# mayataka/robotoc

Measured on NVIDIA H100. Metric: SQP-iterations/s (ANYmal N=40, batch=1024) at 1/2/4/8 H100 vs CPU ref, higher is better.
Workload: dtype f64

## Files before the change

robotoc_b200/csrc/riccati_forward.cuh:

```cuda
#pragma once
#include "rbt_device.cuh"
#include "../../include/rbt_layout.h"

namespace rbt {

struct FwdParams {
  rbt_layout L;
  const rbt_stage_ctrl* ctrl;
  int n_grid;
  int batch;
  const double* kkt;
  const double* ric;
  const double* dx0;
  double* dir;
  int segs;
  const double* dxseed;
  const int* tp_fail;
};

template <int NV, int NU, int NS>
struct FwdCfg {
  static constexpr int NX = 2 * NV;
  static constexpr int NTHREADS = 96;
  static constexpr int KPART = NX * NX + ((NV * NU + 1) & ~1) + ((NX + 1) & ~1);
  static constexpr int RPART = NX * NX + ((NX + 1) & ~1) + ((NU * NX + 1) & ~1) + ((NU + 1) & ~1);
  static constexpr int e_M = 0;
  static constexpr int e_m = e_M + ((NS * NX + 1) & ~1);
  static constexpr int e_Psi = e_m + ((NS + 1) & ~1);
  static constexpr int e_Phi = e_Psi + ((NX + 1) & ~1);
  static constexpr int e_T = e_Phi + ((NX + 1) & ~1);
  static constexpr int e_W = e_T + ((NU + 1) & ~1);
  static constexpr int e_mt = e_W + ((NU + 1) & ~1);
  static constexpr int e_mtn = e_mt + ((NS + 1) & ~1);
  static constexpr int e_pol = e_mtn + ((NS + 1) & ~1);
  static constexpr int e_fx = e_pol + ((NX + 1) & ~1) + 2;
  static constexpr int ESZ = e_fx + ((NX + 1) & ~1);
  static constexpr int SLOT = KPART + RPART + ESZ;
  static constexpr int o_dx = 2 * SLOT;
  static constexpr int o_du = o_dx + 2 * NX;
  static constexpr int o_sc = o_du + ((NU + 1) & ~1);
  static constexpr int o_bar = o_sc + 4;
  static constexpr int SMEM_DOUBLES = o_bar + 4;
  static constexpr size_t SMEM_BYTES = size_t(SMEM_DOUBLES) * 8;
};

template <int NV, int NU, int NS, bool SEG = false>
__global__ void __launch_bounds__(FwdCfg<NV, NU, NS>::NTHREADS, 3) riccati_forward_kernel(const FwdParams p) {
  using C = FwdCfg<NV, NU, NS>;
  constexpr int NX = C::NX, NTHR = C::NTHREADS;
  constexpr int CO = ((NX + 15) / 16) * 16;
  static_assert(CO + NX <= NTHR, "costate thread group must fit");
  extern __shared__ __align__(16) double smem[];
  const rbt_layout& L = p.L;
  const int tid = threadIdx.x;
  const int b = SEG ? int(blockIdx.x) / p.segs : int(blockIdx.x);
  if (b >= p.batch) return;
  const int N = p.n_grid - 1;
  int lo = 0, last = N, seg = 0;
  if constexpr (SEG) {
    seg = int(blockIdx.x) % p.segs;
    if (p.tp_fail[b] != 0) {
      if (seg != 0) return;
    } else {
      lo = tp_seg_lo(seg, N, p.segs);
      last = (seg == p.segs - 1) ? N : tp_seg_lo(seg + 1, N, p.segs) - 1;
    }
  }
  const double* kkt_b = p.kkt + size_t(b) * p.n_grid * L.k_stride;
  const double* ric_b = p.ric + size_t(b) * p.n_grid * L.r_stride;
  double* dir_b = p.dir + size_t(b) * p.n_grid * L.d_stride;
  double* sdx = smem + C::o_dx;
  double* sdu = smem + C::o_du;
  double* ssc = smem + C::o_sc;
  uint64_t* bars = reinterpret_cast<uint64_t*>(smem + C::o_bar);

  auto needs_pol = [&](int st) {
    const rbt_stage_ctrl c = p.ctrl[st];
    return (st == 0 && c.sto) || ((c.type == RBT_IMPACT || c.type == RBT_LIFT) && c.sto_next);
  };
  auto has_extras = [&](int st) {
    const rbt_stage_ctrl c = p.ctrl[st];
    return c.ns > 0 || c.sto || needs_pol(st);
  };
  auto issue = [&](int st) {
    const int slot = (st - lo) & 1;
    double* base = smem + slot * C::SLOT;
    const rbt_stage_ctrl c = p.ctrl[st];
    const double* krec = kkt_b + size_t(st) * L.k_stride;
    const double* rrec = ric_b + size_t(st) * L.r_stride;
    fence_proxy_async();
    if (st < N) {
      mbar_expect_tx(&bars[slot], uint32_t(C::KPART + C::RPART) * 8u);
      tma_load_1d(base, krec + L.k_Fxx, uint32_t(C::KPART) * 8u, &bars[slot]);
      tma_load_1d(base + C::KPART, rrec + L.r_P, uint32_t(C::RPART) * 8u, &bars[slot]);
    } else {
      const uint32_t by = uint32_t(NX * NX + ((NX + 1) & ~1)) * 8u;
      mbar_expect_tx(&bars[slot], by);
      tma_load_1d(base + C::KPART, rrec + L.r_P, by, &bars[slot]);
    }
    if (st < N && has_extras(st)) {
      double* ex = base + C::KPART + C::RPART;
      uint32_t bytes = 0;
      if (c.ns > 0) bytes += uint32_t(C::e_Psi - C::e_M) * 8u;
      if (c.sto) bytes += uint32_t(C::e_mt - C::e_Psi) * 8u + uint32_t(C::ESZ - C::e_fx) * 8u;
      if (c.sto && c.ns > 0) bytes += uint32_t(C::e_pol - C::e_mt) * 8u;
      if (needs_pol(st)) bytes += uint32_t(C::e_fx - C::e_pol) * 8u;
      mbar_expect_tx(&bars[2 + slot], bytes);
      if (c.ns > 0) tma_load_1d(ex + C::e_M, rrec + L.r_M, uint32_t(C::e_Psi - C::e_M) * 8u, &bars[2 + slot]);
      if (c.sto) {
        tma_load_1d(ex + C::e_Psi, rrec + L.r_Psi, uint32_t(C::e_mt - C::e_Psi) * 8u, &bars[2 + slot]);
        tma_load_1d(ex + C::e_fx, krec + L.k_fx, uint32_t(C::ESZ - C::e_fx) * 8u, &bars[2 + slot]);
      }
      if (c.sto && c.ns > 0) tma_load_1d(ex + C::e_mt, rrec + L.r_mt, uint32_t(C::e_pol - C::e_mt) * 8u, &bars[2 + slot]);
      if (needs_pol(st)) tma_load_1d(ex + C::e_pol, rrec + L.r_dtsdx, uint32_t(C::e_fx - C::e_pol) * 8u, &bars[2 + slot]);
    }
  };

  if (tid == 0) {
    for (int q = 0; q < 4; ++q) mbar_init(&bars[q], 1);
    fence_mbar_init();
  }
  if (tid < NX) sdx[tid] = (SEG && lo > 0) ? p.dxseed[(size_t(b) * p.segs + seg) * NX + tid] : p.dx0[size_t(b) * NX + tid];
  if (tid == 0) {
    ssc[0] = 0.0;
    ssc[1] = 0.0;
  }
  __syncthreads();
  if (tid == 0) {
    issue(lo);
    if (last >= lo + 1) issue(lo + 1);
  }
  uint32_t pe0 = 0, pe1 = 0;

  for (int i = lo; i <= last; ++i) {
    const int slot = (i - lo) & 1;
    const rbt_stage_ctrl c = p.ctrl[i];
    const double* base = smem + slot * C::SLOT;
    const double* sA = base;
    const double* sB = base + NX * NX;
    const double* sFx = sB + ((NV * NU + 1) & ~1);
    const double* sPm = base + C::KPART;
    const double* ss = sPm + NX * NX;
    const double* sKt = ss + ((NX + 1) & ~1);
    const double* sk = sKt + ((NU * NX + 1) & ~1);
    const double* ex = base + C::KPART + C::RPART;
    double* dx = sdx + ((i - lo) & 1) * NX;
    double* dxn = sdx + ((i - lo + 1) & 1) * NX;
    double* drec = dir_b + size_t(i) * L.d_stride;
    const bool terminal = (i == N);
    const bool impact = (!terminal && c.type == RBT_IMPACT);
    const bool lift = (!terminal && c.type == RBT_LIFT);
    const bool sto = !terminal && c.sto, sto_next = !terminal && c.sto_next;
    const bool extras = !terminal && has_extras(i);

    mbar_wait(&bars[slot], uint32_t((i - lo) >> 1) & 1u);
    if (extras) {
      if (slot) {
        mbar_wait(&bars[3], pe1);
        pe1 ^= 1;
      } else {
        mbar_wait(&bars[2], pe0);
        pe0 ^= 1;
      }
    }

    double dts = ssc[0], dtsn = ssc[1];
    if (i == 0 && sto) {
      dtsn = dot_serial(ex + C::e_pol, dx, NX) + ex[C::e_pol + ((NX + 1) & ~1) + 1];
    }
    if (lift) {
      dts = dtsn;
      dtsn = 0.0;
      if (sto_next) {
        dtsn = dot_serial(ex + C::e_pol, dx, NX) + ex[C::e_pol + ((NX + 1) & ~1) + 1];
        if (sto) dtsn += ex[C::e_pol + ((NX + 1) & ~1)] * dts;
      }
    }
    if (impact) {
      dts = dtsn;
      dtsn = 0.0;
    }
    const double delta = dtsn - dts;

    if (!terminal && !impact) {
      matvec_T(sKt, NX, NX, NU, dx, tid, NTHR, [&](int u, double a) {
        double v = a + sk[u];
        if (sto) {
          v += ex[C::e_T + u] * delta;
          if (sto_next) v -= ex[C::e_W + u] * dtsn;
        }
        sdu[u] = v;
        drec[L.d_du + u] = v;
      });
      __syncthreads();
    }
    if (tid < NX) {
      const int r = tid;
      drec[L.d_dx + r] = dx[r];
      if (!terminal) {
        double a = sFx[r];
        for (int k = 0; k < NX; ++k) a = fma(sA[r + k * NX], dx[k], a);
        if (!impact) {
          if (r >= NV)
            for (int u = 0; u < NU; ++u) a = fma(sB[(r - NV) + u * NV], sdu[u], a);
          if (sto) a = fma(ex[C::e_fx + r], delta, a);
        }
        dxn[r] = a;
      }
    } else if (tid >= CO && tid < CO + NX && !(impact && sto_next)) {
      const int r = tid - CO;
      double a = -ss[r];
      for (int k = 0; k < NX; ++k) a = fma(sPm[r + k * NX], dx[k], a);
      if (sto) {
        if (impact) {
          a -= ex[C::e_Phi + r] * dtsn;
        } else {
          a += ex[C::e_Psi + r] * delta;
          if (sto_next) a -= ex[C::e_Phi + r] * dtsn;
        }
      }
      drec[L.d_dlmdgmm + r] = a;
    }
    __syncthreads();

    if (impact && sto_next) {
      const double e_dts = dts;
      double e_dtsn = dot_serial(ex + C::e_pol, dxn, NX) + ex[C::e_pol + ((NX + 1) & ~1) + 1];
      if (sto) e_dtsn += ex[C::e_pol + ((NX + 1) & ~1)] * e_dts;
      dts = e_dts;
      dtsn = e_dtsn;
      if (tid >= CO && tid < CO + NX) {
        const int r = tid - CO;
        double a = -ss[r];
        for (int k = 0; k < NX; ++k) a = fma(sPm[r + k * NX], dx[k], a);
        if (sto) a -= ex[C::e_Phi + r] * dtsn;
        drec[L.d_dlmdgmm + r] = a;
      }
    }
    if (!terminal && !impact && c.ns > 0) {
      const int ns = c.ns;
      for (int q = tid; q < ns; q += NTHR) {
        double a = ex[C::e_m + q];
        for (int k = 0; k < NX; ++k) a = fma(ex[C::e_M + q + k * ns], dx[k], a);
        if (sto) {
          a += ex[C::e_mt + q] * delta;
          if (sto_next) a -= ex[C::e_mtn + q] * dtsn;
        }
        drec[L.d_dxi + q] = a;
      }
    }
    if (tid == 0) {
      drec[L.d_dts + 0] = dts;
      drec[L.d_dts + 1] = dtsn;
    }
    __syncthreads();
    if (tid == 0) {
      ssc[0] = dts;
      ssc[1] = dtsn;
      if (i + 2 <= last) issue(i + 2);
    }
    __syncthreads();
  }
}

}
```

robotoc_b200/csrc/stage_kernels.cuh:

```cuda
#pragma once
#include "rbt_device.cuh"
#include "riccati_backward.cuh"
#include "../../include/rbt_stage_layout.h"

namespace rbt {

#define RBT_MAX_TARGETS 96
struct StageParams {
  rbt_layout K;
  rbt_stage_layout S;
  rbt_constraint_table tab;
  const rbt_stage_ctrl* ctrl;
  int n_grid;
  int batch;
  const double* lin;
  double* con;
  double* kkt;
  double* ex;
  double* dir;
  double* xd;
  double* sol;
  double* steps;
  int* info;
  const int4* tgt;
// ... 694 lines not shown
          if (j < 6) v = make_double2(-FiS[r0 + j * 6], -FiS[r0 + 1 + j * 6]);
          else if (j >= NV && j < NV + 6 && !impact) v = make_double2(-dt * Fi[r0 + (j - NV) * 6], -dt * Fi[r0 + 1 + (j - NV) * 6]);
          *reinterpret_cast<double2*>(Fcol + j * NX) = v;
        }
      } else {
        const double dtv = impact ? 0.0 : dt;
#pragma unroll 2
        for (int j = j0; j < NX; j += CP)
          *reinterpret_cast<double2*>(Fcol + j * NX) = make_double2((j == r0) ? 1.0 : ((j == r0 + NV) ? dtv : 0.0),
                                                                    (j == r0 + 1) ? 1.0 : ((j == r0 + 1 + NV) ? dtv : 0.0));
      }
    }
  }
  if (!impact)
    for (int e = tid; e < NV * NU; e += NTHR) kkt[K.k_Fvu + e] = dt * sZ[(e % NV) + (np + e / NV) * NVF];
  for (int ii = tid; ii < NX; ii += NTHR) {
    auto Fxv = [&](int l) { return l >= NV ? vFx[l] - sdt * vr[l - NV] : vFx[l]; };
    double v = Fxv(ii), f = impact ? 0.0 : vfx[ii];
    if (np == 6 && ii < 6) {
      double a1 = 0.0, a2 = 0.0;
      for (int l = 0; l < 6; ++l) {
        a1 = fma(Fi[ii + l * 6], vFx[l], a1);
        a2 = fma(Fi[ii + l * 6], impact ? 0.0 : vfx[l], a2);
      }
      v = -a1;
      f = -a2;
    }
    kkt[K.k_Fx + ii] = v;
    if (!impact) kkt[K.k_fx + ii] = f / c.ngrids_in_phase;
  }
  if (ns > 0) {
    const double* Phia = lin + S.l_Phia;
#pragma unroll 1
    for (int e = tid; e < ns * NV; e += NTHR) ex[S.e_Phia + e] = Phia[e];
#pragma unroll 1
    for (int e = tid; e < ns * NX; e += NTHR) {
      const int q = e % ns, j = e / ns;
      double acc = 0.0;
#pragma unroll 2
      for (int l = 0; l < NV; ++l) acc = fma(Phia[q + l * ns], sR[l + j * NVF], acc);
      kkt[K.k_Phix + e] = lin[S.l_Phix + e] - acc;
    }
#pragma unroll 1
    for (int e = tid; e < ns * NU; e += NTHR) {
      const int q = e % ns, j = e / ns;
      double acc = 0.0;
#pragma unroll 2
      for (int l = 0; l < NV; ++l) acc = fma(Phia[q + l * ns], sZ[l + (np + j) * NVF], acc);
      kkt[K.k_Phiu + e] = acc;
    }
#pragma unroll 1
    for (int q = tid; q < ns; q += NTHR) {
      double acc = 0.0;
#pragma unroll 2
      for (int l = 0; l < NV; ++l) acc = fma(Phia[q + l * ns], vr[l], acc);
      kkt[K.k_p + q] = lin[S.l_p + q] - acc;
      kkt[K.k_Phit + q] = (lin[S.l_Phit + q] - acc) / c.ngrids_in_phase;
    }
  }
  if (!impact && (c.sto || c.sto_next)) {
    const double g1 = 1.0 / c.ngrids_in_phase;
    matvec_T(sR, NVF, NVF, NX, vhaf, tid, NTHR, [&](int ii, double a) {
      double v = vhx[ii] - a;
      if (ii < NV) {
        double a2 = 0.0;
        for (int l = 0; l < NFM; ++l) a2 = fma(sQqf[ii + l * NV], vr[NV + l], a2);
        v += a2 / dt;
      }
      kkt[K.k_hx + ii] = v * g1;
    });
    for (int ii = tid; ii < NU; ii += NTHR) {
      double acc = 0.0;
#pragma unroll 1
      for (int l = 0; l < NVF; ++l) acc = fma(sZ[(np + ii) + l * NVF], vhaf[l], acc);
      kkt[K.k_hu + ii] = (vhu[ii] + acc) * g1;
    }
    if (tid == NTHR - 1) {
      double h = vsc[0];
      for (int l = 0; l < NVF; ++l) h = fma(-vr[l], vhaf[l], h);
      const double Qtt = vsc[1] * g1 * g1;
      kkt[K.k_sc + 0] = Qtt;
      kkt[K.k_sc + 1] = -Qtt;
      kkt[K.k_sc + 2] = h * g1;
      kkt[K.k_sc + 3] = 0.0;
    }
  }
  if (tid == 0) tma_store_wait_read();
}

struct WireParams {
  const rbt_wire_layout* W;
  int n_grid, l_stride;
  long long ocp_stride;
  const double* wire;
  double* lin;
  const double* res;
  double* con;
  int c_stride, c_res, ncp;
};

__global__ void __launch_bounds__(128) unpack_wire_kernel(const WireParams p) {
  const int i = int(blockIdx.x % p.n_grid);
  const size_t b = blockIdx.x / p.n_grid;
  const rbt_wire_layout& W = p.W[i];
  const double* wire = p.wire + b * size_t(p.ocp_stride) + W.ocp_off;
  double* lin = p.lin + size_t(blockIdx.x) * p.l_stride;
  const int nseg = W.nseg;
  for (int k = 0; k < W.nzero; ++k)
    for (int e = threadIdx.x; e < W.zero[k].n; e += 128) lin[W.zero[k].lin_off + e] = 0.0;
  __syncthreads();
  for (int k = 0; k < nseg; ++k) {
    const rbt_wire_seg g = W.seg[k];
    const double* src = wire + g.wire_off;
    double* dst = lin + g.lin_off;
    if (!g.sym) {
      if (g.ld == g.rows) {
        for (int e = threadIdx.x; e < g.rows * g.cols; e += 128) dst[e] = src[e];
      } else {
        for (int e = threadIdx.x; e < g.rows * g.cols; e += 128) dst[(e % g.rows) + (e / g.rows) * g.ld] = src[e];
      }
    } else if (g.sym == 2) {
      for (int e = threadIdx.x; e < g.rows; e += 128) dst[e * (g.ld + 1)] = src[e];
    } else {
      for (int e = threadIdx.x; e < g.rows * g.rows; e += 128) {
        const int r = e % g.rows, c = e / g.rows;
        dst[r + c * g.ld] = (r <= c) ? src[c * (c + 1) / 2 + r] : src[r * (r + 1) / 2 + c];
      }
    }
  }
  if (p.res) {
    const double* r = p.res + size_t(blockIdx.x) * p.ncp;
    double* c = p.con + size_t(blockIdx.x) * p.c_stride + p.c_res;
    for (int e = threadIdx.x; e < p.ncp; e += 128) c[e] = r[e];
  }
}

__global__ void __launch_bounds__(64) pack_slack_dual_kernel(const double* con, int c_stride, int c_slack, int n2, double* out) {
  const double* c = con + size_t(blockIdx.x) * c_stride + c_slack;
  double* o = out + size_t(blockIdx.x) * n2;
  for (int e = threadIdx.x; e < n2; e += 64) o[e] = c[e];
}

__device__ __forceinline__ double warp_min(double v) {
#pragma unroll
  for (int o = 16; o > 0; o >>= 1) v = fmin(v, __shfl_xor_sync(0xffffffffu, v, o));
  return v;
}
__device__ __forceinline__ void atomic_min_pos(double* addr, double v) {
  atomicMin(reinterpret_cast<unsigned long long*>(addr), static_cast<unsigned long long>(__double_as_longlong(v)));
}

constexpr int XTHR = 128;

#ifndef RBT_EXP_MIN_CTAS
#define RBT_EXP_MIN_CTAS 10
#endif
template <int NV, int NU, int NFM>
__global__ void __launch_bounds__(XTHR, RBT_EXP_MIN_CTAS) expand_kernel(const StageParams p) {
  constexpr int NX = 2 * NV, NVF = NV + NFM, NTHR = XTHR;
  constexpr int RSZ = ((NVF * NX + 1) & ~1) + ((NVF + 1) & ~1);
  constexpr int ZSZ = NVF * NU;
  __shared__ __align__(16) double sR[RSZ];
  __shared__ __align__(16) double sZ[ZSZ];
  __shared__ __align__(16) double sG[512];
  __shared__ __align__(16) double sC[4 * 160];
  __shared__ double sdx[NX], sdu[NU], sdaf[NVF], spart[4][32], smin[8];
  __shared__ __align__(8) uint64_t bar;
  const rbt_layout& K = p.K;
  const rbt_stage_layout& S = p.S;
  const int tid = threadIdx.x, lane = tid & 31, wid = tid >> 5;
  const size_t o = blockIdx.x;
  const int i = int(o % p.n_grid), b = int(o / p.n_grid);
  const rbt_stage_ctrl c = p.ctrl[i];
  if (c.type == RBT_TERMINAL) return;
  const bool impact = (c.type == RBT_IMPACT);
  const bool pdipm = !impact || p.tab.impact_friction_cone != 0;
  constexpr int np = NV - NU;
  const int nf = c.nf, nvf = NV + nf;
  const double* lin = p.lin + o * S.l_stride;
  const double* ex = p.ex + o * S.e_stride;
  const double* d = p.dir + o * K.d_stride;
  double* con = p.con + o * S.c_stride;
  double* xd = p.xd + o * S.x_stride;
  const int gsz = S.l_stride - S.l_dgdq;
  if (tid == 0) {
    mbar_init(&bar, 1);
    fence_mbar_init();
    uint32_t bytes = RSZ * 8;
    if (!impact) bytes += ZSZ * 8;
    if (pdipm) bytes += gsz * 8 + 4 * S.ncp * 8;
    mbar_expect_tx(&bar, bytes);
    tma_load_1d(sR, ex + S.e_R, RSZ * 8, &bar);
    if (!impact) tma_load_1d(sZ, ex + S.e_Z + np * NVF, ZSZ * 8, &bar);
    if (pdipm) {
      tma_load_1d(sG, lin + S.l_dgdq, gsz * 8, &bar);
      tma_load_1d(sC, con + S.c_slack, 4 * S.ncp * 8, &bar);
    }
  }
  for (int e = tid; e < NX; e += NTHR) sdx[e] = d[K.d_dx + e];
  for (int e = tid; e < NU; e += NTHR) sdu[e] = impact ? 0.0 : d[K.d_du + e];
  const int nbox = p.tab.n_box, ncp = S.ncp;
  __syncthreads();
  mbar_wait(&bar, 0);
  {
    double acc = 0.0;
    if (lane < nvf) {
      for (int k = wid; k < NX; k += 4) acc = fma(-sR[lane + k * NVF], sdx[k], acc);
      if (!impact)
        for (int k = wid; k < NU; k += 4) acc = fma(sZ[lane + k * NVF], sdu[k], acc);
    }
    spart[wid][lane] = acc;
  }
  __syncthreads();
  if (tid < nvf) {
    double acc = (spart[0][tid] + spart[1][tid]) + (spart[2][tid] + spart[3][tid]);
    acc -= sR[((NVF * NX + 1) & ~1) + tid];
    if (tid >= NV) acc = -acc;
    sdaf[tid] = acc;
    xd[S.x_daf + tid] = acc;
  }
  if (!pdipm) return;
  __syncthreads();
  const double tau = p.tab.fraction_to_boundary;
  double mp = 1.0, md = 1.0;
  for (int r = tid; r < S.nc; r += NTHR) {
    if (r < nbox && (impact || __ldg(p.row_level + r) + c.ineq_gate > 2)) continue;
    const double c_sl = sC[r], c_du = sC[ncp + r], c_res = sC[2 * ncp + r], c_cm = sC[3 * ncp + r];
    double dsl, ddu;
    if (r < nbox) {
      const rbt_box_row br = p.tab.box[r];
      const double var = br.var == RBT_VAR_Q ? sdx[br.idx] : br.var == RBT_VAR_V ? sdx[NV + br.idx]
                         : br.var == RBT_VAR_A ? sdaf[br.idx] : sdu[br.idx];
      dsl = -br.sign * var - c_res;
      ddu = -(c_du * dsl + c_cm) / c_sl;
    } else {
      const int q = r - nbox, ci = q / 5, r5 = q % 5;
      dsl = 1.0; ddu = 1.0;
      if ((c.contact_mask >> ci) & 1) {
        const int fstack = 3 * __popc(c.contact_mask & ((1 << ci) - 1));
        const double* dgdq = sG + size_t(ci) * 5 * NV;
        const double* dgdf = sG + (S.l_dgdf - S.l_dgdq) + size_t(ci) * 15;
        double a0 = 0.0, a1 = 0.0;
        for (int j = 0; j < NV; j += 2) {
          a0 = fma(dgdq[r5 + j * 5], sdx[j], a0);
          if (j + 1 < NV) a1 = fma(dgdq[r5 + (j + 1) * 5], sdx[j + 1], a1);
        }
        double acc = a0 + a1;
        for (int j = 0; j < 3; ++j) acc = fma(dgdf[r5 + j * 5], sdaf[NV + fstack + j], acc);
        dsl = -acc - c_res;
        ddu = -(c_du * dsl + c_cm) / c_sl;
      }
    }
    con[S.c_dslack + r] = dsl;
    con[S.c_ddual + r] = ddu;
    const double fp = -tau * (c_sl / dsl), fd = -tau * (c_du / ddu);
    if (fp > 0.0 && fp < 1.0) mp = fmin(mp, fp);
    if (fd > 0.0 && fd < 1.0) md = fmin(md, fd);
  }
  mp = warp_min(mp);
  md = warp_min(md);
  if (lane == 0) {
    smin[wid * 2] = mp;
    smin[wid * 2 + 1] = md;
  }
  __syncthreads();
  if (tid == 0) {
    atomic_min_pos(&p.steps[2 * b], fmin(fmin(smin[0], smin[2]), fmin(smin[4], smin[6])));
    atomic_min_pos(&p.steps[2 * b + 1], fmin(fmin(smin[1], smin[3]), fmin(smin[5], smin[7])));
  }
}

__device__ __forceinline__ void integrate_free_flyer_dev(double* q, const double* dq, double step) {
  const double vx = step * dq[0], vy = step * dq[1], vz = step * dq[2];
  const double wx = step * dq[3], wy = step * dq[4], wz = step * dq[5];
  const double th2 = wx * wx + wy * wy + wz * wz, th = sqrt(th2);
  double bb, cc, s2 = 0.0, c2 = 1.0;
  if (th < 1e-6) {
    bb = 0.5 - th2 / 24.0; cc = 1.0 / 6.0 - th2 / 120.0;
  } else {
    sincos(0.5 * th, &s2, &c2);
    bb = 2.0 * s2 * s2 / th2; cc = (th - 2.0 * s2 * c2) / (th2 * th);
  }
  const double cx = wy * vz - wz * vy, cy = wz * vx - wx * vz, cz = wx * vy - wy * vx;
  const double ccx = wy * cz - wz * cy, ccy = wz * cx - wx * cz, ccz = wx * cy - wy * cx;
  const double tx = vx + bb * cx + cc * ccx, ty = vy + bb * cy + cc * ccy, tz = vz + bb * cz + cc * ccz;
  const double qx = q[3], qy = q[4], qz = q[5], qw = q[6];
  const double ux = qy * tz - qz * ty, uy = qz * tx - qx * tz, uz = qx * ty - qy * tx;
  const double u2x = qy * uz - qz * uy, u2y = qz * ux - qx * uz, u2z = qx * uy - qy * ux;
  q[0] += tx + 2.0 * (qw * ux + u2x);
  q[1] += ty + 2.0 * (qw * uy + u2y);
  q[2] += tz + 2.0 * (qw * uz + u2z);
  double sh, ch;
  if (th < 1e-6) { sh = 0.5 - th2 / 48.0; ch = 1.0 - th2 / 8.0; } else { sh = s2 / th; ch = c2; }
  const double ex_ = sh * wx, ey = sh * wy, ez = sh * wz, ew = ch;
  const double nx_ = qw * ex_ + qx * ew + qy * ez - qz * ey;
  const double ny = qw * ey - qx * ez + qy * ew + qz * ex_;
  const double nz = qw * ez + qx * ey - qy * ex_ + qz * ew;
  const double nw = qw * ew - qx * ex_ - qy * ey - qz * ez;
  const double nrm = 1.0 / sqrt(nx_ * nx_ + ny * ny + nz * nz + nw * nw);
  q[3] = nx_ * nrm; q[4] = ny * nrm; q[5] = nz * nrm; q[6] = nw * nrm;
}

#ifndef RBT_UPD_MIN_CTAS
#define RBT_UPD_MIN_CTAS 12
#endif
template <int NV, int NU, int NFM>
__global__ void __launch_bounds__(XTHR, RBT_UPD_MIN_CTAS) update_kernel(const StageParams p) {
  constexpr int NX = 2 * NV, NVF = NV + NFM, NTHR = XTHR;
  constexpr int QSZ = NFM * NX + NFM * NV + ((NV + 1) & ~1);
  constexpr int ZSZ = (NVF * NVF + 1) & ~1;
  constexpr int PSZ = ((NX * 6 + 1) & ~1) + ((6 * NU + 1) & ~1) + 6;
  __shared__ __align__(16) double sQ[QSZ];
  __shared__ __align__(16) double sZ[ZSZ];
  __shared__ __align__(16) double sP[PSZ];
  __shared__ double sdx[NX], sdu[NU], slaf[NVF], sdl[NX], sdgn[NV], spart[4][32];
  __shared__ __align__(8) uint64_t bar;
  const rbt_layout& K = p.K;
  const rbt_stage_layout& S = p.S;
  const int tid = threadIdx.x, lane = tid & 31, wid = tid >> 5;
  const size_t o = blockIdx.x;
  const int i = int(o % p.n_grid), b = int(o / p.n_grid);
  const rbt_stage_ctrl c = p.ctrl[i];
  const bool terminal = (c.type == RBT_TERMINAL), impact = (c.type == RBT_IMPACT);
  constexpr int np = NV - NU;
  const int nf = terminal ? 0 : c.nf, nvf = NV + nf, ns = (terminal || impact) ? 0 : c.ns;
  double* ex = p.ex + o * S.e_stride;
  double* d = p.dir + o * K.d_stride;
  double* xd = p.xd + o * S.x_stride;
  double* con = p.con + o * S.c_stride;
  double* sol = p.sol + o * S.s_stride;
  const bool nup = !terminal && !impact && np == 6;
  if (tid == 0 && !terminal) {
    mbar_init(&bar, 1);
    fence_mbar_init();
    mbar_expect_tx(&bar, (QSZ + ZSZ + (nup ? PSZ : 0)) * 8);
    tma_load_1d(sQ, ex + S.e_Qaf, QSZ * 8, &bar);
    tma_load_1d(sZ, ex + S.e_Z, ZSZ * 8, &bar);
    if (nup) tma_load_1d(sP, ex + S.e_Qxup, PSZ * 8, &bar);
  }
  const double ap = p.steps[2 * b], ad = p.steps[2 * b + 1];
  for (int e = tid; e < NX; e += NTHR) {
    sdx[e] = d[K.d_dx + e];
    sdl[e] = d[K.d_dlmdgmm + e];
  }
  for (int e = tid; e < NU; e += NTHR) sdu[e] = (terminal || impact) ? 0.0 : d[K.d_du + e];
  if (!terminal)
    for (int e = tid; e < NV; e += NTHR) sdgn[e] = d[K.d_stride + K.d_dlmdgmm + NV + e];
  if (!terminal && (!impact || p.tab.impact_friction_cone != 0)) {
    for (int r = tid + (impact ? p.tab.n_box : 0); r < S.nc; r += NTHR) {
      if (r < p.tab.n_box && __ldg(p.row_level + r) + c.ineq_gate > 2) continue;
      con[S.c_slack + r] += ap * con[S.c_dslack + r];
      con[S.c_dual + r] += ad * con[S.c_ddual + r];
    }
  }
  __syncthreads();
  if (np == 6) {
    if (tid == 2 * 32) integrate_free_flyer_dev(sol + S.s_q, sdx, ap);
    if (tid < 6) {
      double acc = 0.0;
      for (int l = 0; l < 6; ++l) acc = fma(ex[S.e_Fqqpi + l + tid * 6], sdl[l], acc);
      d[K.d_dlmdgmm + tid] = -acc;
      sol[S.s_lmd + tid] += ap * (-acc);
    }
  }
  for (int e = tid; e < NV; e += NTHR) {
    if (np == 6) {
      if (e >= 6) {
        sol[S.s_q + e + 1] += ap * sdx[e];
        sol[S.s_lmd + e] += ap * sdl[e];
      }
    } else {
      sol[S.s_q + e] += ap * sdx[e];
      sol[S.s_lmd + e] += ap * sdl[e];
    }
    sol[S.s_v + e] += ap * sdx[NV + e];
    sol[S.s_gmm + e] += ap * sdl[NV + e];
    if (!terminal) {
      const double da = xd[S.x_daf + e];
      if (!impact) {
        sol[S.s_a + e] += ap * da;
        sol[S.s_dv + e] = 0.0;
      } else {
        sol[S.s_a + e] = 0.0;
        sol[S.s_dv + e] += ap * da;
      }
    }
  }
  if (terminal) return;
  for (int e = tid; e < NU; e += NTHR) sol[S.s_u + e] = impact ? 0.0 : sol[S.s_u + e] + ap * sdu[e];
  for (int e = tid; e < nf; e += NTHR) sol[S.s_f + e] += ap * xd[S.x_daf + NV + e];
  for (int e = tid; e < ns; e += NTHR) sol[S.s_xi + e] += ap * d[K.d_dxi + e];
  const double dt = c.dt;
  double dts = 0.0;
  if (!impact && c.ngrids_in_phase > 0) dts = (d[K.d_dts + 1] - d[K.d_dts]) / c.ngrids_in_phase;
  const double bm_old = (tid < nvf) ? (tid < NV ? sol[S.s_beta + tid] : sol[S.s_mu + tid - NV]) : 0.0;
  const double nup_old = (nup && wid == 3 && (lane >> 2) < 6 && (lane & 3) == 0) ? sol[S.s_nup + (lane >> 2)] : 0.0;
  double extra = 0.0;
  if (tid < nvf) {
    extra = ex[S.e_laf + tid];
    if (!impact) {
      if (tid < NV) {
        extra = fma(dt, sdgn[tid], extra);
        for (int q = 0; q < ns; ++q) extra = fma(ex[S.e_Phia + q + tid * ns], d[K.d_dxi + q], extra);
      }
      if (dts < -2.220446049250313e-16 || dts > 2.220446049250313e-16) extra = fma(dts, ex[S.e_haf + tid], extra);
    } else if (tid < NV) {
      extra += sdgn[tid];
    }
  }
  const double da_r = (tid < NV) ? xd[S.x_daf + tid] + ex[S.e_r + tid] : 0.0;
  mbar_wait(&bar, 0);
  if (tid < NV) extra = fma(sQ[NFM * NX + NFM * NV + tid], da_r, extra);
  {
    double acc = 0.0;
    if (lane >= NV && lane < nvf) {
      const double* q = sQ + (lane - NV);
      for (int k = wid; k < NX; k += 4) acc = fma(q[k * NFM], sdx[k], acc);
      if (!impact) {
        const double* qu = q + NFM * NX + np * NFM;
        for (int k = wid; k < NU; k += 4) acc = fma(qu[k * NFM], sdu[k], acc);
      }
    }
    spart[wid][lane] = acc;
  }
  if (nup && wid == 3) {
    const int prow = lane >> 2, ppart = lane & 3;
    const double* sQxup = sP;
    const double* sQuup = sP + ((NX * 6 + 1) & ~1);
    const double* slup = sQuup + ((6 * NU + 1) & ~1);
    double pn = 0.0;
    if (prow < 6) {
      for (int k = ppart; k < NU; k += 4) pn = fma(-sQuup[prow + k * 6], sdu[k], pn);
      for (int k = ppart; k < NX; k += 4) pn = fma(-sQxup[k + prow * NX], sdx[k], pn);
      for (int k = ppart; k < NV; k += 4) pn = fma(-dt * sZ[prow + k * NVF], sdgn[k], pn);
    }
    pn += __shfl_xor_sync(0xffffffffu, pn, 1);
    pn += __shfl_xor_sync(0xffffffffu, pn, 2);
    if (prow < 6 && ppart == 0) {
      pn -= slup[prow];
      xd[S.x_dnup + prow] = pn;
      sol[S.s_nup + prow] = nup_old + ap * pn;
    }
  }
  __syncthreads();
  if (tid < nvf) {
    const double acc = extra + ((spart[0][tid] + spart[1][tid]) + (spart[2][tid] + spart[3][tid]));
    slaf[tid] = acc;
    ex[S.e_laf + tid] = acc;
  }
  __syncthreads();
  {
    double acc = 0.0;
    if (lane < nvf)
      for (int k = wid; k < nvf; k += 4) acc = fma(-sZ[lane + k * NVF], slaf[k], acc);
    spart[wid][lane] = acc;
  }
  __syncthreads();
  if (tid < nvf) {
    const double acc = (spart[0][tid] + spart[1][tid]) + (spart[2][tid] + spart[3][tid]);
    xd[S.x_dbetamu + tid] = acc;
    if (tid < NV) sol[S.s_beta + tid] = bm_old + ap * acc;
    else sol[S.s_mu + tid - NV] = bm_old + ap * acc;
  }
}

}
```

Baseline: 208,300.

## Shrink forward-pass smem ring, reuse opposite slot for extras, restructure update loads

The Riccati forward kernel drops the separate extras region and extras barriers. It loads a stage's extras into the other ring slot, so the prefetch depth falls to one stage when extras are present. The dts and dtsn scalars move to registers, and one of the two per-stage __syncthreads is removed when there are no extras. This shrinks shared memory so four blocks can share an SM. The update kernel is restructured so that each warp preloads the old solution values it owns into registers before the barrier, issuing all global loads early rather than doing serial read-modify-write; its min-CTA launch bound is lowered from 12 to 8.

```diff
diff --git a/robotoc_b200/csrc/riccati_forward.cuh b/robotoc_b200/csrc/riccati_forward.cuh
--- a/robotoc_b200/csrc/riccati_forward.cuh
+++ b/robotoc_b200/csrc/riccati_forward.cuh
@@ -35,17 +35,17 @@
   static constexpr int e_pol = e_mtn + ((NS + 1) & ~1);
   static constexpr int e_fx = e_pol + ((NX + 1) & ~1) + 2;
   static constexpr int ESZ = e_fx + ((NX + 1) & ~1);
-  static constexpr int SLOT = KPART + RPART + ESZ;
+  static constexpr int SLOT = KPART + RPART;
+  static_assert(ESZ <= SLOT, "the extras of a stage must fit one ring slot");
   static constexpr int o_dx = 2 * SLOT;
   static constexpr int o_du = o_dx + 2 * NX;
-  static constexpr int o_sc = o_du + ((NU + 1) & ~1);
-  static constexpr int o_bar = o_sc + 4;
-  static constexpr int SMEM_DOUBLES = o_bar + 4;
+  static constexpr int o_bar = o_du + ((NU + 1) & ~1);
+  static constexpr int SMEM_DOUBLES = o_bar + 2;
   static constexpr size_t SMEM_BYTES = size_t(SMEM_DOUBLES) * 8;
 };
 
 template <int NV, int NU, int NS, bool SEG = false>
-__global__ void __launch_bounds__(FwdCfg<NV, NU, NS>::NTHREADS, 3) riccati_forward_kernel(const FwdParams p) {
+__global__ void __launch_bounds__(FwdCfg<NV, NU, NS>::NTHREADS, 4) riccati_forward_kernel(const FwdParams p) {
   using C = FwdCfg<NV, NU, NS>;
   constexpr int NX = C::NX, NTHR = C::NTHREADS;
   constexpr int CO = ((NX + 15) / 16) * 16;
@@ -71,7 +71,6 @@
   double* dir_b = p.dir + size_t(b) * p.n_grid * L.d_stride;
   double* sdx = smem + C::o_dx;
   double* sdu = smem + C::o_du;
-  double* ssc = smem + C::o_sc;
   uint64_t* bars = reinterpret_cast<uint64_t*>(smem + C::o_bar);
 
   auto needs_pol = [&](int st) {
@@ -80,12 +79,11 @@
   };
   auto has_extras = [&](int st) {
     const rbt_stage_ctrl c = p.ctrl[st];
-    return c.ns > 0 || c.sto || needs_pol(st);
-  };
-  auto issue = [&](int st) {
+    return st < N && (c.ns > 0 || c.sto || needs_pol(st));
+  };
+  auto issue_main = [&](int st) {
     const int slot = (st - lo) & 1;
     double* base = smem + slot * C::SLOT;
-    const rbt_stage_ctrl c = p.ctrl[st];
     const double* krec = kkt_b + size_t(st) * L.k_stride;
     const double* rrec = ric_b + size_t(st) * L.r_stride;
     fence_proxy_async();
@@ -98,39 +96,47 @@
       mbar_expect_tx(&bars[slot], by);
       tma_load_1d(base + C::KPART, rrec + L.r_P, by, &bars[slot]);
     }
-    if (st < N && has_extras(st)) {
-      double* ex = base + C::KPART + C::RPART;
-      uint32_t bytes = 0;
-      if (c.ns > 0) bytes += uint32_t(C::e_Psi - C::e_M) * 8u;
-      if (c.sto) bytes += uint32_t(C::e_mt - C::e_Psi) * 8u + uint32_t(C::ESZ - C::e_fx) * 8u;
-      if (c.sto && c.ns > 0) bytes += uint32_t(C::e_pol - C::e_mt) * 8u;
-      if (needs_pol(st)) bytes += uint32_t(C::e_fx - C::e_pol) * 8u;
-      mbar_expect_tx(&bars[2 + slot], bytes);
-      if (c.ns > 0) tma_load_1d(ex + C::e_M, rrec + L.r_M, uint32_t(C::e_Psi - C::e_M) * 8u, &bars[2 + slot]);
-      if (c.sto) {
-        tma_load_1d(ex + C::e_Psi, rrec + L.r_Psi, uint32_t(C::e_mt - C::e_Psi) * 8u, &bars[2 + slot]);
-        tma_load_1d(ex + C::e_fx, krec + L.k_fx, uint32_t(C::ESZ - C::e_fx) * 8u, &bars[2 + slot]);
-      }
-      if (c.sto && c.ns > 0) tma_load_1d(ex + C::e_mt, rrec + L.r_mt, uint32_t(C::e_pol - C::e_mt) * 8u, &bars[2 + slot]);
-      if (needs_pol(st)) tma_load_1d(ex + C::e_pol, rrec + L.r_dtsdx, uint32_t(C::e_fx - C::e_pol) * 8u, &bars[2 + slot]);
-    }
+  };
+  auto issue_extras = [&](int st) {
+    const int slot = (st - lo + 1) & 1;
+    double* ex = smem + slot * C::SLOT;
+    const rbt_stage_ctrl c = p.ctrl[st];
+    const double* krec = kkt_b + size_t(st) * L.k_stride;
+    const double* rrec = ric_b + size_t(st) * L.r_stride;
+    fence_proxy_async();
+    uint32_t bytes = 0;
+    if (c.ns > 0) bytes += uint32_t(C::e_Psi - C::e_M) * 8u;
+    if (c.sto) bytes += uint32_t(C::e_mt - C::e_Psi) * 8u + uint32_t(C::ESZ - C::e_fx) * 8u;
+    if (c.sto && c.ns > 0) bytes += uint32_t(C::e_pol - C::e_mt) * 8u;
+    if (needs_pol(st)) bytes += uint32_t(C::e_fx - C::e_pol) * 8u;
+    mbar_expect_tx(&bars[slot], bytes);
+    if (c.ns > 0) tma_load_1d(ex + C::e_M, rrec + L.r_M, uint32_t(C::e_Psi - C::e_M) * 8u, &bars[slot]);
+    if (c.sto) {
+      tma_load_1d(ex + C::e_Psi, rrec + L.r_Psi, uint32_t(C::e_mt - C::e_Psi) * 8u, &bars[slot]);
+      tma_load_1d(ex + C::e_fx, krec + L.k_fx, uint32_t(C::ESZ - C::e_fx) * 8u, &bars[slot]);
+    }
+    if (c.sto && c.ns > 0) tma_load_1d(ex + C::e_mt, rrec + L.r_mt, uint32_t(C::e_pol - C::e_mt) * 8u, &bars[slot]);
+    if (needs_pol(st)) tma_load_1d(ex + C::e_pol, rrec + L.r_dtsdx, uint32_t(C::e_fx - C::e_pol) * 8u, &bars[slot]);
+  };
+  auto issue_after = [&](int i) {
+    if (has_extras(i) && i + 1 <= last) issue_main(i + 1);
+    if (i + 1 <= last && has_extras(i + 1)) issue_extras(i + 1);
+    else if (i + 2 <= last) issue_main(i + 2);
   };
 
   if (tid == 0) {
-    for (int q = 0; q < 4; ++q) mbar_init(&bars[q], 1);
+    for (int q = 0; q < 2; ++q) mbar_init(&bars[q], 1);
     fence_mbar_init();
   }
   if (tid < NX) sdx[tid] = (SEG && lo > 0) ? p.dxseed[(size_t(b) * p.segs + seg) * NX + tid] : p.dx0[size_t(b) * NX + tid];
-  if (tid == 0) {
-    ssc[0] = 0.0;
-    ssc[1] = 0.0;
-  }
   __syncthreads();
   if (tid == 0) {
-    issue(lo);
-    if (last >= lo + 1) issue(lo + 1);
-  }
-  uint32_t pe0 = 0, pe1 = 0;
+    issue_main(lo);
+    if (has_extras(lo)) issue_extras(lo);
+    else if (last >= lo + 1) issue_main(lo + 1);
+  }
+  uint32_t ph = 0;
+  double dts = 0.0, dtsn = 0.0;
 
   for (int i = lo; i <= last; ++i) {
     const int slot = (i - lo) & 1;
@@ -143,7 +149,7 @@
     const double* ss = sPm + NX * NX;
     const double* sKt = ss + ((NX + 1) & ~1);
     const double* sk = sKt + ((NU * NX + 1) & ~1);
-    const double* ex = base + C::KPART + C::RPART;
+    const double* ex = smem + (slot ^ 1) * C::SLOT;
     double* dx = sdx + ((i - lo) & 1) * NX;
     double* dxn = sdx + ((i - lo + 1) & 1) * NX;
     double* drec = dir_b + size_t(i) * L.d_stride;
@@ -153,18 +159,13 @@
     const bool sto = !terminal && c.sto, sto_next = !terminal && c.sto_next;
     const bool extras = !terminal && has_extras(i);
 
-    mbar_wait(&bars[slot], uint32_t((i - lo) >> 1) & 1u);
+    mbar_wait(&bars[slot], (ph >> slot) & 1u);
+    ph ^= 1u << slot;
     if (extras) {
-      if (slot) {
-        mbar_wait(&bars[3], pe1);
-        pe1 ^= 1;
-      } else {
-        mbar_wait(&bars[2], pe0);
-        pe0 ^= 1;
-      }
-    }
-
-    double dts = ssc[0], dtsn = ssc[1];
+      mbar_wait(&bars[slot ^ 1], (ph >> (slot ^ 1)) & 1u);
+      ph ^= 1u << (slot ^ 1);
+    }
+
     if (i == 0 && sto) {
       dtsn = dot_serial(ex + C::e_pol, dx, NX) + ex[C::e_pol + ((NX + 1) & ~1) + 1];
     }
@@ -223,43 +224,40 @@
     }
     __syncthreads();
 
-    if (impact && sto_next) {
-      const double e_dts = dts;
-      double e_dtsn = dot_serial(ex + C::e_pol, dxn, NX) + ex[C::e_pol + ((NX + 1) & ~1) + 1];
-      if (sto) e_dtsn += ex[C::e_pol + ((NX + 1) & ~1)] * e_dts;
-      dts = e_dts;
-      dtsn = e_dtsn;
-      if (tid >= CO && tid < CO + NX) {
-        const int r = tid - CO;
-        double a = -ss[r];
-        for (int k = 0; k < NX; ++k) a = fma(sPm[r + k * NX], dx[k], a);
-        if (sto) a -= ex[C::e_Phi + r] * dtsn;
-        drec[L.d_dlmdgmm + r] = a;
-      }
-    }
-    if (!terminal && !impact && c.ns > 0) {
-      const int ns = c.ns;
-      for (int q = tid; q < ns; q += NTHR) {
-        double a = ex[C::e_m + q];
-        for (int k = 0; k < NX; ++k) a = fma(ex[C::e_M + q + k * ns], dx[k], a);
-        if (sto) {
-          a += ex[C::e_mt + q] * delta;
-          if (sto_next) a -= ex[C::e_mtn + q] * dtsn;
-        }
-        drec[L.d_dxi + q] = a;
-      }
+    if (extras) {
+      if (impact && sto_next) {
+        const double e_dts = dts;
+        double e_dtsn = dot_serial(ex + C::e_pol, dxn, NX) + ex[C::e_pol + ((NX + 1) & ~1) + 1];
+        if (sto) e_dtsn += ex[C::e_pol + ((NX + 1) & ~1)] * e_dts;
+        dts = e_dts;
+        dtsn = e_dtsn;
+        if (tid >= CO && tid < CO + NX) {
+          const int r = tid - CO;
+          double a = -ss[r];
+          for (int k = 0; k < NX; ++k) a = fma(sPm[r + k * NX], dx[k], a);
+          if (sto) a -= ex[C::e_Phi + r] * dtsn;
+          drec[L.d_dlmdgmm + r] = a;
+        }
+      }
+      if (!terminal && !impact && c.ns > 0) {
+        const int ns = c.ns;
+        for (int q = tid; q < ns; q += NTHR) {
+          double a = ex[C::e_m + q];
+          for (int k = 0; k < NX; ++k) a = fma(ex[C::e_M + q + k * ns], dx[k], a);
+          if (sto) {
+            a += ex[C::e_mt + q] * delta;
+            if (sto_next) a -= ex[C::e_mtn + q] * dtsn;
+          }
+          drec[L.d_dxi + q] = a;
+        }
+      }
+      __syncthreads();
     }
     if (tid == 0) {
       drec[L.d_dts + 0] = dts;
       drec[L.d_dts + 1] = dtsn;
-    }
-    __syncthreads();
-    if (tid == 0) {
-      ssc[0] = dts;
-      ssc[1] = dtsn;
-      if (i + 2 <= last) issue(i + 2);
-    }
-    __syncthreads();
+      issue_after(i);
+    }
   }
 }
 
diff --git a/robotoc_b200/csrc/stage_kernels.cuh b/robotoc_b200/csrc/stage_kernels.cuh
--- a/robotoc_b200/csrc/stage_kernels.cuh
+++ b/robotoc_b200/csrc/stage_kernels.cuh
@@ -1020,11 +1020,12 @@
 }
 
 #ifndef RBT_UPD_MIN_CTAS
-#define RBT_UPD_MIN_CTAS 12
+#define RBT_UPD_MIN_CTAS 8
 #endif
 template <int NV, int NU, int NFM>
 __global__ void __launch_bounds__(XTHR, RBT_UPD_MIN_CTAS) update_kernel(const StageParams p) {
   constexpr int NX = 2 * NV, NVF = NV + NFM, NTHR = XTHR;
+  static_assert(NVF <= 32 && NX <= NTHR, "one lane per row");
   constexpr int QSZ = NFM * NX + NFM * NV + ((NV + 1) & ~1);
   constexpr int ZSZ = (NVF * NVF + 1) & ~1;
   constexpr int PSZ = ((NX * 6 + 1) & ~1) + ((6 * NU + 1) & ~1) + 6;
@@ -1057,76 +1058,136 @@
     if (nup) tma_load_1d(sP, ex + S.e_Qxup, PSZ * 8, &bar);
   }
   const double ap = p.steps[2 * b], ad = p.steps[2 * b + 1];
-  for (int e = tid; e < NX; e += NTHR) {
-    sdx[e] = d[K.d_dx + e];
-    sdl[e] = d[K.d_dlmdgmm + e];
-  }
-  for (int e = tid; e < NU; e += NTHR) sdu[e] = (terminal || impact) ? 0.0 : d[K.d_du + e];
-  if (!terminal)
-    for (int e = tid; e < NV; e += NTHR) sdgn[e] = d[K.d_stride + K.d_dlmdgmm + NV + e];
+
+  double ov[10];
+#pragma unroll
+  for (int l = 0; l < 10; ++l) ov[l] = 0.0;
+  const bool w0 = wid == 0 && !terminal && lane < nvf;
+  const bool sto_dts = !impact && c.ngrids_in_phase > 0;
+  double &e_laf = ov[0], &bm_old = ov[1], &da_r = ov[2], &dts_n = ov[3], &dts_0 = ov[4];
+  if (w0) {
+    e_laf = ex[S.e_laf + lane];
+    bm_old = lane < NV ? sol[S.s_beta + lane] : sol[S.s_mu + lane - NV];
+    if (lane < NV) da_r = xd[S.x_daf + lane] + ex[S.e_r + lane];
+    if (sto_dts) {
+      dts_n = d[K.d_dts + 1];
+      dts_0 = d[K.d_dts];
+    }
+  }
+  const bool w1 = wid == 1 && lane < NV;
+  const bool cc = w1 && np == 6 && lane < 6;
+  const int qrow = (np == 6) ? lane + 1 : lane;
+  double &q_old = ov[0], &lmd_old = ov[1], &v_old = ov[2], &gmm_old = ov[3];
+  double* fqq = ov + 4;
+  if (w1) {
+    if (!cc) q_old = sol[S.s_q + qrow];
+    lmd_old = sol[S.s_lmd + lane];
+    v_old = sol[S.s_v + lane];
+    gmm_old = sol[S.s_gmm + lane];
+    if (cc)
+#pragma unroll
+      for (int l = 0; l < 6; ++l) fqq[l] = ex[S.e_Fqqpi + l + lane * 6];
+  }
+  const bool w2 = wid == 2 && !terminal;
+  double &a_old = ov[0], &da = ov[1], &u_old = ov[2], &f_old = ov[3], &df = ov[4];
+  if (w2) {
+    if (lane < NV) {
+      da = xd[S.x_daf + lane];
+      a_old = impact ? sol[S.s_dv + lane] : sol[S.s_a + lane];
+    }
+    if (lane < NU && !impact) u_old = sol[S.s_u + lane];
+    if (lane < nf) {
+      f_old = sol[S.s_f + lane];
+      df = xd[S.x_daf + NV + lane];
+    }
+  }
+  const bool ff = np == 6 && tid == 3 * 32 + 31;
+  const bool w3 = wid == 3 && lane < ns;
+  double* qff = ov;
+  double &xi_old = ov[7], &dxi = ov[8], &nup_old = ov[9];
+  if (ff)
+#pragma unroll
+    for (int l = 0; l < 7; ++l) qff[l] = sol[S.s_q + l];
+  if (w3) {
+    xi_old = sol[S.s_xi + lane];
+    dxi = d[K.d_dxi + lane];
+  }
+  if (nup && wid == 3 && (lane >> 2) < 6 && (lane & 3) == 0) nup_old = sol[S.s_nup + (lane >> 2)];
+  double x_dx = 0.0, x_dl = 0.0, x_du = 0.0, x_dgn = 0.0;
+  if (tid < NX) {
+    x_dx = d[K.d_dx + tid];
+    x_dl = d[K.d_dlmdgmm + tid];
+  }
+  if (tid < NU && !terminal && !impact) x_du = d[K.d_du + tid];
+  if (tid < NV && !terminal) x_dgn = d[K.d_stride + K.d_dlmdgmm + NV + tid];
+
   if (!terminal && (!impact || p.tab.impact_friction_cone != 0)) {
     for (int r = tid + (impact ? p.tab.n_box : 0); r < S.nc; r += NTHR) {
-      if (r < p.tab.n_box && __ldg(p.row_level + r) + c.ineq_gate > 2) continue;
-      con[S.c_slack + r] += ap * con[S.c_dslack + r];
-      con[S.c_dual + r] += ad * con[S.c_ddual + r];
-    }
-  }
+      const bool skip = r < p.tab.n_box && __ldg(p.row_level + r) + c.ineq_gate > 2;
+      const double sl = con[S.c_slack + r], dsl = con[S.c_dslack + r], du = con[S.c_dual + r], ddu = con[S.c_ddual + r];
+      if (skip) continue;
+      con[S.c_slack + r] = sl + ap * dsl;
+      con[S.c_dual + r] = du + ad * ddu;
+    }
+  }
+  if (tid < NX) {
+    sdx[tid] = x_dx;
+    sdl[tid] = x_dl;
+  }
+  if (tid < NU) sdu[tid] = x_du;
+  if (tid < NV && !terminal) sdgn[tid] = x_dgn;
   __syncthreads();
-  if (np == 6) {
-    if (tid == 2 * 32) integrate_free_flyer_dev(sol + S.s_q, sdx, ap);
-    if (tid < 6) {
+
+  if (ff) {
+    integrate_free_flyer_dev(qff, sdx, ap);
+#pragma unroll
+    for (int l = 0; l < 7; ++l) sol[S.s_q + l] = qff[l];
+  }
+  if (w1) {
+    if (cc) {
       double acc = 0.0;
-      for (int l = 0; l < 6; ++l) acc = fma(ex[S.e_Fqqpi + l + tid * 6], sdl[l], acc);
-      d[K.d_dlmdgmm + tid] = -acc;
-      sol[S.s_lmd + tid] += ap * (-acc);
-    }
-  }
-  for (int e = tid; e < NV; e += NTHR) {
-    if (np == 6) {
-      if (e >= 6) {
-        sol[S.s_q + e + 1] += ap * sdx[e];
-        sol[S.s_lmd + e] += ap * sdl[e];
-      }
+#pragma unroll
+      for (int l = 0; l < 6; ++l) acc = fma(fqq[l], sdl[l], acc);
+      d[K.d_dlmdgmm + lane] = -acc;
+      sol[S.s_lmd + lane] = lmd_old + ap * (-acc);
     } else {
-      sol[S.s_q + e] += ap * sdx[e];
-      sol[S.s_lmd + e] += ap * sdl[e];
-    }
-    sol[S.s_v + e] += ap * sdx[NV + e];
-    sol[S.s_gmm + e] += ap * sdl[NV + e];
-    if (!terminal) {
-      const double da = xd[S.x_daf + e];
+      sol[S.s_q + qrow] = q_old + ap * sdx[lane];
+      sol[S.s_lmd + lane] = lmd_old + ap * sdl[lane];
+    }
+    sol[S.s_v + lane] = v_old + ap * sdx[NV + lane];
+    sol[S.s_gmm + lane] = gmm_old + ap * sdl[NV + lane];
+  }
+  if (terminal) return;
+  if (w2) {
+    if (lane < NV) {
       if (!impact) {
-        sol[S.s_a + e] += ap * da;
-        sol[S.s_dv + e] = 0.0;
+        sol[S.s_a + lane] = a_old + ap * da;
+        sol[S.s_dv + lane] = 0.0;
       } else {
-        sol[S.s_a + e] = 0.0;
-        sol[S.s_dv + e] += ap * da;
-      }
-    }
-  }
-  if (terminal) return;
-  for (int e = tid; e < NU; e += NTHR) sol[S.s_u + e] = impact ? 0.0 : sol[S.s_u + e] + ap * sdu[e];
-  for (int e = tid; e < nf; e += NTHR) sol[S.s_f + e] += ap * xd[S.x_daf + NV + e];
-  for (int e = tid; e < ns; e += NTHR) sol[S.s_xi + e] += ap * d[K.d_dxi + e];
+        sol[S.s_a + lane] = 0.0;
+        sol[S.s_dv + lane] = a_old + ap * da;
+      }
+    }
+    if (lane < NU) sol[S.s_u + lane] = impact ? 0.0 : u_old + ap * sdu[lane];
+    if (lane < nf) sol[S.s_f + lane] = f_old + ap * df;
+  }
+  if (w3) sol[S.s_xi + lane] = xi_old + ap * dxi;
   const double dt = c.dt;
   double dts = 0.0;
-  if (!impact && c.ngrids_in_phase > 0) dts = (d[K.d_dts + 1] - d[K.d_dts]) / c.ngrids_in_phase;
-  const double bm_old = (tid < nvf) ? (tid < NV ? sol[S.s_beta + tid] : sol[S.s_mu + tid - NV]) : 0.0;
-  const double nup_old = (nup && wid == 3 && (lane >> 2) < 6 && (lane & 3) == 0) ? sol[S.s_nup + (lane >> 2)] : 0.0;
+  if (sto_dts) dts = (dts_n - dts_0) / c.ngrids_in_phase;
   double extra = 0.0;
-  if (tid < nvf) {
-    extra = ex[S.e_laf + tid];
+  if (w0) {
+    extra = e_laf;
     if (!impact) {
-      if (tid < NV) {
-        extra = fma(dt, sdgn[tid], extra);
-        for (int q = 0; q < ns; ++q) extra = fma(ex[S.e_Phia + q + tid * ns], d[K.d_dxi + q], extra);
-      }
-      if (dts < -2.220446049250313e-16 || dts > 2.220446049250313e-16) extra = fma(dts, ex[S.e_haf + tid], extra);
-    } else if (tid < NV) {
-      extra += sdgn[tid];
-    }
-  }
-  const double da_r = (tid < NV) ? xd[S.x_daf + tid] + ex[S.e_r + tid] : 0.0;
+      if (lane < NV) {
+        extra = fma(dt, sdgn[lane], extra);
+        for (int q = 0; q < ns; ++q) extra = fma(ex[S.e_Phia + q + lane * ns], d[K.d_dxi + q], extra);
+      }
+      if (dts < -2.220446049250313e-16 || dts > 2.220446049250313e-16) extra = fma(dts, ex[S.e_haf + lane], extra);
+    } else if (lane < NV) {
+      extra += sdgn[lane];
+    }
+  }
   mbar_wait(&bar, 0);
   if (tid < NV) extra = fma(sQ[NFM * NX + NFM * NV + tid], da_r, extra);
   {
```

After: 214,700, median of 6. 1.03x the previous value.
